# iAmLakshya/code-rag

Hardware: AMD Instinct MI355X
Metric: top-k queries/s over 10Mx768 (cosine top-100, batch 64) (higher is better)
Workload: dtype bf16; 1 GPU; 1x MI355X: 10000000x768 bf16 corpus per GPU resident in HBM, batch-64 queries, exact top-100; rows_per_gpu=10000000, dim=768, batch=64, k=100, parallelism=row-shard x1, hbm_resident_bytes_per_row=2308

## Files before the change

code-rag_amd/csrc/crh_i8.hpp:

```cpp
#pragma once

namespace crh {

typedef __attribute__((ext_vector_type(4))) int i32x4;
typedef __attribute__((ext_vector_type(16))) int i32x16;
typedef __attribute__((ext_vector_type(2))) float f32x2;

constexpr int kI8SampleTiles = 8192;
constexpr float kI8QueryLevels = 16256.0f;

#ifdef CRH_ENABLE_DEBUG
struct I8DebugEnds {
    float *hi, *lo;
    long long pitch;
};
__device__ I8DebugEnds g_i8_debug_ends;
#endif

template <bool F32>
__global__ __launch_bounds__(64) void k_requant_i8(const u32x4 *__restrict__ xt, const float *__restrict__ xf32, u32x4 *__restrict__ x8,
                                                   float *__restrict__ srow, unsigned int *__restrict__ dn_bits, int64_t t0, int ksteps,
                                                   int64_t count, u32x4 *__restrict__ xrow)
{
    const int64_t tile = t0 + blockIdx.x;
    const int lane = threadIdx.x, row = lane & 31, hh = lane >> 5;
    const bool live = tile * 32 + row < count;
    const u32x4 *tp = xt + (size_t)tile * ksteps * 64;
    const int ks8 = ksteps >> 1, dim = ksteps * 16;
    const float4 *fr = reinterpret_cast<const float4 *>(xf32 + ((size_t)tile * 32 + row) * dim);
    auto fetch16 = [&](int p, float (&v)[16], bool copy_row) {
        if (!live) {
#pragma unroll
// ... 117 lines not shown
    }
}

__device__ __forceinline__ uint32_t bf16_bits_up(float x)
{
    const uint32_t u = f32_bits(x);
    return (u >> 31) ? (u >> 16) : ((u + 0xffffu) >> 16);
}
__device__ __forceinline__ int nonsample_tile(int p, int G, int S)
{
    const int per = S - 1, full = G * per;
    if (p >= full) return G * S + (p - full);
    const int blk = p / per;
    return blk * S + 1 + (p - blk * per);
}

template <int KS8, int WAVES, int RING, int QB, int PART>
__global__ __launch_bounds__(WAVES * 64) void k_scan_i8(
    const u32x4 *__restrict__ x8, const float *__restrict__ srow, const unsigned int *__restrict__ dn_bits,
    const u32x4 *__restrict__ qfrag8, const float *__restrict__ qpar, const uint32_t *__restrict__ rowmask, int ntiles, int G, int S,
    uint32_t *__restrict__ gkey, float *__restrict__ tau_g, int k, float c_abs, float sqrt_dim, int nq, u32x4 *__restrict__ wave_lists,
    int wave_cap, unsigned int *__restrict__ qcount, u32x2 *__restrict__ qlist, float *__restrict__ qlo, int qcap,
    SearchStatus *__restrict__ status, const u32x4 *__restrict__ xt, const float *__restrict__ xf32,
    const float *__restrict__ qn, const u32x4 *__restrict__ xrow, u32x4 *__restrict__ shi = nullptr)
{
    static_assert(PART >= 1 && PART <= 3, "sample tiles / thresholds / pass");
    static_assert(KS8 % RING == 0, "the ring must divide the pieces of a tile (slot s % RING holds piece s of every tile)");
    constexpr int NT = WAVES * 64, NQS = QB * 32, NB = NT < 1024 ? NT : 1024;
    __shared__ u32x4 qs[QB * 2 * KS8 * 64];
    __shared__ uint32_t col[kI8SampleTiles];
    __shared__ unsigned int hist[(NT / 64) * 256];
    __shared__ unsigned int bcast[2];
    __shared__ unsigned int fast[NB + 256 + 2 * (NT / 64) + 8];
    __shared__ float tau_s[NQS];
    __shared__ unsigned int qcnt_l[64];
    __shared__ unsigned int wpre[WAVES + 1];
    __shared__ unsigned int wcnt_l[WAVES];
    __shared__ float hwf[64];
    __shared__ int next_m;
    __shared__ unsigned long long cslot[8];
    __shared__ int next_g;
    const int tid = threadIdx.x;
    const int lane = tid & 63;
    const int wave = __builtin_amdgcn_readfirstlane(tid >> 6);
    const int h = lane >> 5;

    CRH_STAMP(0);
    if (tid < 64) qcnt_l[tid] = 0u;
    if (tid < WAVES) wcnt_l[tid] = 0u;
    if (tid == 0) {
        next_m = WAVES;
        next_g = WAVES;
        if constexpr (PART == 3) {
            for (int j = 2; j < 8; ++j) cslot[j] = ~0ull;
            cslot[0] = (unsigned long long)blockIdx.x;
            cslot[1] = (1ull << 32) | (gridDim.x + __hip_atomic_fetch_add(&status->next_chunk, 1u, __ATOMIC_RELAXED, __HIP_MEMORY_SCOPE_AGENT));
        }
// ... 153 lines not shown
                uint32_t m = 0u;
#pragma unroll
                for (int r = 0; r < 16; ++r) {
                    const int row = (r & 3) + 8 * (r >> 2) + 4 * h;
                    const uint32_t key = (ord_f32(lower_end(hi[b][r], sr, b, r)) & ~31u) | (uint32_t)row;
                    m = max(m, ((vmask >> row) & 1u) ? key : 0u);
                }
                m = max(m, (uint32_t)__shfl_xor((int)m, 32));
                if (h == 0) gkey[(size_t)(b * 32 + lane) * G + g] = m;
            }
            g = gn_;
        }
        asm volatile("s_waitcnt vmcnt(0)" ::: "memory");
        return;
    }

    constexpr unsigned int kFloorKey = 0x007fffffu;
    constexpr int SELCAP = 384;
    static_assert(NB + 256 + 2 * (NT / 64) + 8 >= 2 * SELCAP, "sel / selv overlay the scratch of wg_kth_largest_fast");
    static_assert((NT / 64) * 256 >= KS8 * 32, "the canonical query overlays the radix histograms");
    if constexpr (PART == 2)
    for (int q = blockIdx.x; q < NQS; q += gridDim.x) {
        float t = -INFINITY;
        if (q >= nq) {
            t = INFINITY;
        } else if (G >= k) {
            constexpr int DIM = KS8 * 32;
            float qreg[(DIM + NT - 1) / NT];
#pragma unroll
            for (int j = 0; j < (DIM + NT - 1) / NT; ++j) qreg[j] = (tid + j * NT < DIM) ? qn[(size_t)q * DIM + tid + j * NT] : 0.f;
            {
                constexpr int PER = kI8SampleTiles / NT;
                uint32_t kreg[PER];
#pragma unroll
                for (int j = 0; j < PER; ++j) kreg[j] = (tid + j * NT < G) ? gkey[(size_t)q * G + tid + j * NT] : 0u;
#pragma unroll
                for (int j = 0; j < PER; ++j)
                    if (tid + j * NT < G) col[tid + j * NT] = kreg[j];
            }
            __syncthreads();
            CRH_TAU_STAMP(8);
            const uint32_t key = wg_kth_largest_fast<NT, NB, 256>([&](unsigned int i) { return col[i]; }, (unsigned int)G, (unsigned int)k,
                                                                  kFloorKey, fast, hist, bcast);
            __syncthreads();
            CRH_TAU_STAMP(9);
            if (key > kFloorKey) {
// ... 19 lines not shown
                if (nsel <= (unsigned int)SELCAP) {
                    const int sub = tid & 7;
                    for (unsigned int r0 = 0; r0 < nsel; r0 += NT / 8) {
                        const unsigned int r = r0 + (unsigned int)(tid >> 3);
                        float acc = 0.f;
                        if (r < nsel) {
                            const uint32_t e = sel[r];
                            acc = partial_dot8<6>(xt, xf32, xrow, DIM, KS8 * 2, (uint32_t)((e >> 5) * (uint32_t)S * 32u + (e & 31u)), qv, sub);
                        }
                        acc = sum8(acc);
                        if (r < nsel && sub == 0) selv[r] = acc;
                    }
                    __syncthreads();
                    CRH_TAU_STAMP(11);
                    if ((unsigned int)tid < nsel) {
                        const float v = selv[tid];
                        unsigned int gt = 0u, ge = 0u;
                        for (unsigned int j = 0; j < nsel; ++j) {
                            const float o = selv[j];
                            gt += o > v ? 1u : 0u;
                            ge += o >= v ? 1u : 0u;
                        }
                        if (gt < (unsigned int)k && (unsigned int)k <= ge) bcast[1] = f32_bits(v);
                    }
                    __syncthreads();
                    CRH_TAU_STAMP(12);
                    t = fmaxf(t, bits_f32(bcast[1]) - c_abs);
                }
            }
            __syncthreads();
        }
        if (tid == 0) tau_g[q] = t;
    }
    if constexpr (PART == 2) return;
    const bool stored = shi != nullptr;
    const int npass = stored ? ntiles - G : ntiles;
    auto order = [&](int p) { return stored ? nonsample_tile(p, G, S) : p; };
    if (gw < npass) prime(tile_ptr(order(gw)));
    for (int i = tid; i < QB * 2 * KS8 * 64; i += NT) qs[i] = qfrag8[i];
    CRH_STAMP(5);
    if (tid < NQS) tau_s[tid] = tau_g[tid];
    __syncthreads();
    float tq[QB];
#pragma unroll
    for (int b = 0; b < QB; ++b) tq[b] = tau_s[b * 32 + (lane & 31)];

    auto emit_tile = [&](int64_t tile, uint32_t vmask, const float (&hi)[QB][16], uint32_t rounded) __attribute__((always_inline)) {
        uint32_t pmask = 0u;
#pragma unroll
        for (int b = 0; b < QB; ++b)
#pragma unroll
            for (int r = 0; r < 16; ++r) pmask |= (hi[b][r] >= tq[b]) ? (1u << (b * 16 + r)) : 0u;
        {
            const uint32_t t = vmask >> (4 * h);
            const uint32_t v16 = (t & 0xfu) | ((t >> 4) & 0xf0u) | ((t >> 8) & 0xf00u) | ((t >> 12) & 0xf000u);
            pmask &= v16 | (v16 << 16);
        }
#if defined(CRH_I8_DBG) && CRH_I8_DBG == 2
        asm volatile("" ::"v"(pmask));
        pmask = 0u;
#endif
        if (pmask != 0u) {
            const uint32_t rowbase = (uint32_t)(tile * 32) + 4u * (uint32_t)h;
            unsigned int pos = atomicAdd(&wcnt_l[wave], (unsigned int)__popc(pmask));
            uint32_t m = pmask;
            do {
                const int bit = __builtin_ctz(m);
                m &= m - 1u;
                float hv = hi[0][0];
#pragma unroll
                for (int b = 0; b < QB; ++b)
#pragma unroll
                    for (int rr = 0; rr < 16; ++rr) hv = (bit == b * 16 + rr) ? hi[b][rr] : hv;
                const int r = bit & 15;
                if (pos < (unsigned int)wave_cap) {
                    u32x4 e;
                    e.x = f32_bits(hv);
                    e.y = rowbase + (uint32_t)((r & 3) + 8 * (r >> 2));
                    e.z = (uint32_t)((bit >> 4) * 32 + (lane & 31));
                    e.w = rounded;
                    mylist[pos] = e;
                    atomicAdd(&qcnt_l[e.z], 1u);
                }
                ++pos;
            } while (m != 0u);
        }
    };
    if (stored) {
        for (int g = gw; g < G; g += total) {
            float hi[QB][16];
#pragma unroll
            for (int b = 0; b < QB; ++b)
#pragma unroll
                for (int v = 0; v < 2; ++v) {
                    const u32x4 pk = shi[((size_t)g * (QB * 2) + b * 2 + v) * 64 + lane];
                    const uint32_t w4[4] = {pk.x, pk.y, pk.z, pk.w};
#pragma unroll
                    for (int e = 0; e < 4; ++e) {
                        hi[b][8 * v + 2 * e] = bits_f32(w4[e] << 16);
                        hi[b][8 * v + 2 * e + 1] = bits_f32(w4[e] & 0xffff0000u);
                    }
                }
            const int64_t tile = (int64_t)g * S;
            emit_tile(tile, rowmask[tile], hi, 1u);
        }
    }
    int i = gw;
    const u32x4 *xp = tile_ptr(i < npass ? order(i) : 0);
    while (i < npass) {
#if !defined(CRH_I8_STATIC)
        int inext_l = 0;
        if (lane == 0) {
            const int m = atomicAdd(&next_m, 1);
            const unsigned int j = (unsigned int)(m / WAVES), w = (unsigned int)(m % WAVES);
            if (w == 0) {
                const unsigned int c = gridDim.x + __hip_atomic_fetch_add(&status->next_chunk, 1u, __ATOMIC_RELAXED, __HIP_MEMORY_SCOPE_AGENT);
                __hip_atomic_store(&cslot[(j + 1) % 8], ((unsigned long long)(j + 1) << 32) | c, __ATOMIC_RELAXED, __HIP_MEMORY_SCOPE_WORKGROUP);
            }
            unsigned long long e;
            while (((e = __hip_atomic_load(&cslot[j % 8], __ATOMIC_RELAXED, __HIP_MEMORY_SCOPE_WORKGROUP)) >> 32) != j) __builtin_amdgcn_s_sleep(1);
            const unsigned int c = (unsigned int)e;
            inext_l = c > 0x7fffffffu / WAVES ? 0x7fffffff : (int)(c * WAVES + w);
        }
        const int inext = __builtin_amdgcn_readfirstlane(inext_l);
#else
        const int inext = i + total;
#endif
        const int64_t tile = order(i);
        const u32x4 *xn = (inext < npass) ? tile_ptr(order(inext)) : xp;
        const uint32_t vmask = rowmask[tile];
        float sr[32];
#pragma unroll
        for (int j = 0; j < 32; ++j) sr[j] = srow[(size_t)tile * 32 + j];
        i32x16 acc[QB][2];
        scan_tile(xp, xn, acc);
        float hi[QB][16];
        intervals(acc, sr, hi);
        emit_tile(tile, vmask, hi, 0u);
        xp = xn;
        i = inext;
    }
    asm volatile("s_waitcnt vmcnt(0)" ::: "memory");
    CRH_STAMP(6);
#ifdef CRH_FUSED_STAMPS
    if (lane == 0 && blockIdx.x < 256 && wave < 16) g_fused_stamps[256 * 8 + blockIdx.x * 16 + wave] = wall_clock64();
#endif

    if (lane == 0) {
        const unsigned int wcnt = wcnt_l[wave];
        wpre[wave + 1] = wcnt < (unsigned int)wave_cap ? wcnt : (unsigned int)wave_cap;
        atomicMax(&status->max_wave_cnt, wcnt);
        if (wcnt > (unsigned int)wave_cap) atomicAdd(&status->wave_overflow, 1u);
    }
    __syncthreads();
    unsigned int *base = reinterpret_cast<unsigned int *>(qs);
    unsigned int *off = base + 64;
    if (tid < 64) {
        const unsigned int n = qcnt_l[tid];
        base[tid] = n ? atomicAdd(&qcount[tid], n) : 0u;
        off[tid] = 0u;
    }
// ... 24 lines not shown
        }
#pragma unroll
        for (int j = 0; j < 8; ++j) {
            const unsigned int e = e0 + j * NT;
            s_r[j] = e < nall ? srow[cnd[j].y] : 0.f;
        }
#pragma unroll
        for (int j = 0; j < 8; ++j) {
            const unsigned int e = e0 + j * NT;
            if (e < nall) {
                const unsigned int q = cnd[j].z & 63u;
                const unsigned int idx = base[q] + atomicAdd(&off[q], 1u);
                if (idx < (unsigned int)qcap) {
                    u32x2 o;
                    o.x = cnd[j].x;
                    o.y = cnd[j].y;
                    qlist[(size_t)q * qcap + idx] = o;
                    const float up = bits_f32(cnd[j].x);
                    qlo[(size_t)q * qcap + idx] = up - 2.0f * fmaf(s_r[j], hwf[q], c_abs) - 2e-6f - (cnd[j].w ? fabsf(up) * (1.0f / 128.0f) : 0.f);
                }
            }
        }
    }
#ifdef CRH_FUSED_STAMPS
    __syncthreads();
    CRH_STAMP(7);
#endif
}

}
```

code-rag_amd/csrc/crh_index.hip:

```cpp
#include <algorithm>
#include <chrono>
#include <cmath>
#include <cstdlib>
#include <cstring>
#include <vector>

#include "crh_common.h"
#include "crh_kernels.hpp"
#include "crh_i8.hpp"
#include "crh_range.hpp"

namespace crh {
std::string &last_error_ref()
{
    thread_local std::string s;
    return s;
}
}

using namespace crh;

namespace {

constexpr int kWaves = 16;
// ... 46 lines not shown

}

struct crh_index {
    int dim = 0, ksteps = 0, dtype = 0, ncols = 0, device = 0, cu_count = 0;
    int batch_q = 64;
    bool wide_ok = false;
    bool fused_scan = true;
    std::chrono::steady_clock::time_point fused_rest_until{};
    double fused_rest_s = 0.2;
    bool fused_resting() const { return std::chrono::steady_clock::now() < fused_rest_until; }
    bool i8 = false;
    u32x4 *x8 = nullptr;
    float *srow = nullptr;
    u32x4 *xrow = nullptr;
    bool want_xrow = true;
    unsigned int *i8stat = nullptr;
    int64_t x8_cap_tiles = 0, i8_dirty_from = 0;
    int i8_strikes = 0;
    int i8_cooldown = 0;
    bool i8_suppress = false;
    int nominate_max = CRH_NOMINATE_INT8;
    bool i8_sample_record = true;
    bool i8_sample_auto = true;
    int i8_sample = kI8SampleTiles;
    int64_t i8_min_rows = 1000000;
    int64_t cap_rows = 0, cap_tiles = 0, count = 0, alive_count = 0;
    uint64_t mutations = 1;
    MaskCache mask;
    bool sparse_on = true;
    int sparse_den = kSparseDen;
    MaskCache cmask;
    FilterClasses *cmask_classes = nullptr;
    u32x4 *xt = nullptr;
    float *xf32 = nullptr;
    uint32_t *alive = nullptr;
    int32_t *codes = nullptr;
    unsigned int *scratch_u32 = nullptr;

    int seed_tiles = 4096, wave_cap = 2048, qcap = 65536, force_fallback = 0;

    struct Workspace {
        int ws_blocks = 0, ws_wave_cap = 0, ws_qcap = 0, ws_seed = 0;
        int64_t ws_mask_tiles = 0;
        float *qn = nullptr, *gmax = nullptr, *tau = nullptr, *qpar = nullptr, *qlo = nullptr;
        u32x4 *qfrag = nullptr, *qfrag8 = nullptr, *wave_lists = nullptr, *shi = nullptr;
        uint32_t *effmask = nullptr;
        int64_t ws_cmask_tiles = 0;
        uint32_t *cmask = nullptr;
        uint32_t *cunion = nullptr;
        uint32_t *clist = nullptr;
        uint32_t *tilelist = nullptr;
        u32x2 *qlist = nullptr;
        unsigned long long *skeys = nullptr, *skeys2 = nullptr;
    };
    Workspace ws;
    SearchStatus *status = nullptr;
    float *stage_q = nullptr;
    int64_t stage_q_elems = 0;
    float *stage_os = nullptr;
    int64_t *stage_or = nullptr;
    int64_t stage_out_elems = 0;
    unsigned long long *stage_cnt = nullptr;
    int64_t stage_cnt_elems = 0;
    void *stage_in = nullptr;
    int64_t stage_in_bytes = 0;

    std::vector<Pending> pending;
    int next_slot = 0;
// ... 36 lines not shown
    h->stage_in = nullptr;
    h->stage_in_bytes = 0;
    CRH_HIP(hipMalloc(&h->stage_in, (size_t)bytes));
    h->stage_in_bytes = bytes;
    return CRH_OK;
}

int scan_blocks(const crh_index *h, int64_t nitems)
{
    int64_t b = ceil_div(nitems, kWaves);
    if (b > h->cu_count) b = h->cu_count;
    if (b < 1) b = 1;
    return (int)b;
}

int ensure_workspace(crh_index *h, crh_index::Workspace &w, int wave_cap, int qcap)
{
    const int blocks = h->cu_count;
    if (!w.qn) CRH_TRY(dev_alloc(&w.qn, (int64_t)kWideQ * h->dim));
    if (!w.qfrag) CRH_TRY(dev_alloc(&w.qfrag, (int64_t)(kWideQ / 32) * h->ksteps * 64));
    if (!w.tau) CRH_TRY(dev_alloc(&w.tau, kWideQ));
    if (h->i8 && !w.qfrag8) CRH_TRY(dev_alloc(&w.qfrag8, (int64_t)(kMaxQ / 32) * 2 * (h->dim / 32) * 64));
    if (h->i8 && !w.qpar) CRH_TRY(dev_alloc(&w.qpar, kMaxQ * 4));
    if (h->i8 && !w.shi && hipMalloc(reinterpret_cast<void **>(&w.shi), (size_t)kI8SampleTiles * 64 * 4 * sizeof(u32x4)) != hipSuccess) {
        (void)hipGetLastError();
        w.shi = nullptr;
        h->i8_sample_record = false;
    }
    if (!h->status) {
        CRH_TRY(dev_alloc(&h->status, kStatusSlots));
        CRH_HIP(hipMemset(h->status, 0, sizeof(SearchStatus) * kStatusSlots));
    }
    if (w.ws_seed < h->seed_tiles) {
        dev_free(w.gmax);
        w.ws_seed = 0;
        CRH_TRY(dev_alloc(&w.gmax, (int64_t)h->seed_tiles * kWideQ));
        w.ws_seed = h->seed_tiles;
    }
    if (w.ws_mask_tiles < h->cap_tiles) {
        dev_free(w.effmask);
        dev_free(w.tilelist);
        w.ws_mask_tiles = 0;
        h->mask.built_at = 0;
        CRH_TRY(dev_alloc(&w.effmask, h->cap_tiles));
        CRH_TRY(dev_alloc(&w.tilelist, h->cap_tiles + ceil_div(h->cap_tiles, 256) + 1));
        w.ws_mask_tiles = h->cap_tiles;
// ... 365 lines not shown
    }
    return CRH_OK;
}

float i8_c_abs(const crh_index *h) { return 1.5e-4f * (h->dim > 768 ? (float)h->dim / 768.f : 1.f) + 1e-5f; }

void i8_sample_plan(const crh_index *h, int64_t ntiles, int *G, int *S)
{
    int64_t g_auto = h->i8_sample;
    if (h->seed_tiles == 4096 && h->i8_sample_auto)
        g_auto = std::max<int64_t>(1024, std::min<int64_t>(h->i8_sample, (int64_t)(h->i8_sample * std::sqrt((double)ntiles / 312500.0))));
    *G = (int)std::min<int64_t>(h->seed_tiles == 4096 ? g_auto : h->seed_tiles, ntiles);
    *S = (int)std::max<int64_t>(1, ntiles / *G);
}

template <int PART>
int launch_scan_i8(crh_index *h, crh_index::Workspace &w, int blocks, hipStream_t st, const uint32_t *mask, int ntiles, int G, int S, int k, float c_abs,
                   int nq, int wave_cap, int qcap, SearchStatus *stt, u32x4 *shi)
{
#define CRH_I8(KS8, RING, QB)                                                                                                          \
    hipLaunchKernelGGL((k_scan_i8<KS8, kI8Waves, RING, QB, PART>), dim3(PART == 2 ? QB * 32 : blocks), dim3(kI8Waves * 64), 0, st, h->x8, h->srow, \
                       h->i8stat, w.qfrag8, w.qpar, mask, ntiles, G, S, reinterpret_cast<uint32_t *>(w.gmax), w.tau, k, c_abs, sqrtf((float)h->dim), \
                       nq, w.wave_lists, wave_cap, stt->qcount, w.qlist, w.qlo, qcap, stt, h->xt,                                               \
                       h->dtype == CRH_DTYPE_F32 ? h->xf32 : (const float *)nullptr, w.qn, h->xrow, PART == 2 ? (u32x4 *)nullptr : shi)
    switch (h->dim) {
    case 384: CRH_I8(12, 12, 2); break;
    case 768: CRH_I8(24, kI8Ring, 2); break;
    case 1024: CRH_I8(32, kI8Ring, 2); break;
    case 1536: CRH_I8(48, kI8Ring, 1); break;
    default: return fail(CRH_E_INTERNAL, "no int8 scan kernel for dim %d", h->dim);
    }
#undef CRH_I8
    CRH_HIP(hipGetLastError());
    return CRH_OK;
}

template <int MODE>
int launch_scan_wide(crh_index *h, crh_index::Workspace &w, hipStream_t st, const uint32_t *mask, int nitems, int stride, int nblk, int wave_cap, int qcap,
                     SearchStatus *stt)
{
    const int blocks = (int)std::max<int64_t>(1, std::min<int64_t>(nitems, h->cu_count));
#define CRH_WIDE(KS)                                                                                                              \
    hipLaunchKernelGGL((k_scan_wide<KS, MODE>), dim3(blocks), dim3(512), 0, st, h->xt, w.qfrag, w.tau, mask, nitems, stride, nblk, \
                       w.gmax, kWideQ, w.wave_lists, kWideWaves, wave_cap * (kWaves / kWideWaves), stt->qcount, w.qlist, qcap, stt)
    switch (h->ksteps) {
    case 24: CRH_WIDE(24); break;
    case 48: CRH_WIDE(48); break;
// ... 473 lines not shown
    int ndev = 0;
    if (hipGetDeviceCount(&ndev) != hipSuccess || ndev == 0) return fail(CRH_E_NODEVICE, "no HIP device visible");
    if (device < 0 || device >= ndev) return fail(CRH_E_INVALID, "device %d out of range (%d visible)", device, ndev);
    hipDeviceProp_t prop;
    CRH_HIP(hipGetDeviceProperties(&prop, device));
    if (strncmp(prop.gcnArchName, "gfx950", 6) != 0)
        return fail(CRH_E_NODEVICE, "device %d is %s; this library is built for gfx950 only", device, prop.gcnArchName);
    DeviceGuard g(device);
    if (!g.ok) return fail(CRH_E_HIP, "hipSetDevice(%d) failed", device);

    crh_index *h = new crh_index();
    h->dim = dim;
    h->ksteps = dim / 16;
    h->batch_q = dim > 1024 ? 32 : 64;
    h->wide_ok = dim <= 768 && getenv("CODERAG_HIP_NO_WIDE_SCAN") == nullptr;
    {
        const char *e = getenv("CODERAG_HIP_FUSED_SCAN");
        h->fused_scan = !(e && e[0] == '0');
        const char *e8 = getenv("CODERAG_HIP_I8");
        h->i8 = h->fused_scan && !(e8 && e8[0] == '0');
        if (h->i8) h->qcap = 131072;
        if (const char *em = getenv("CODERAG_HIP_I8_MIN_ROWS")) h->i8_min_rows = atoll(em);
        if (const char *er = getenv("CODERAG_HIP_I8_SAMPLE_RECORD")) h->i8_sample_record = !(er[0] == '0');
        if (const char *es = getenv("CODERAG_HIP_I8_SAMPLE")) {
            h->i8_sample = std::max(1024, std::min(kI8SampleTiles, atoi(es)));
            h->i8_sample_auto = false;
        }
        if (const char *er = getenv("CODERAG_HIP_ROWMAJOR")) h->want_xrow = er[0] != '0';
        if (const char *ep = getenv("CODERAG_HIP_SPARSE")) h->sparse_on = ep[0] != '0';
        if (const char *ed = getenv("CODERAG_HIP_SPARSE_DEN")) h->sparse_den = std::max(1, atoi(ed));
    }
    h->dtype = dtype;
    h->ncols = n_code_cols;
    h->device = device;
    h->cu_count = prop.multiProcessorCount;
    h->cap_rows = (capacity_rows + 31) & ~31LL;
    h->cap_tiles = h->cap_rows / 32;
    int rc = dev_alloc(&h->xt, h->cap_tiles * h->ksteps * 64);
    if (rc == CRH_OK && dtype == CRH_DTYPE_F32) rc = dev_alloc(&h->xf32, h->cap_rows * dim);
    if (rc == CRH_OK) rc = dev_alloc(&h->alive, h->cap_tiles);
    if (rc == CRH_OK && n_code_cols) rc = dev_alloc(&h->codes, h->cap_rows * n_code_cols);
    if (rc == CRH_OK) rc = dev_alloc(&h->scratch_u32, 4);
    if (rc == CRH_OK && hipMemset(h->xt, 0, (size_t)h->cap_tiles * h->ksteps * 1024) != hipSuccess) rc = fail(CRH_E_HIP, "hipMemset(xt) failed");
    if (rc == CRH_OK && hipMemset(h->alive, 0, (size_t)h->cap_tiles * 4) != hipSuccess) rc = fail(CRH_E_HIP, "hipMemset(alive) failed");
    if (rc == CRH_OK && h->codes && hipMemset(h->codes, 0xff, (size_t)h->cap_rows * n_code_cols * 4) != hipSuccess)
        rc = fail(CRH_E_HIP, "hipMemset(codes) failed");
// ... 15 lines not shown
    dev_free(h->xf32);
    dev_free(h->alive);
    dev_free(h->codes);
    dev_free(h->scratch_u32);
    dev_free(h->mask.sets);
    dev_free(h->cmask.sets);
    dev_free(h->cmask_classes);
    {
        crh_index::Workspace &w = h->ws;
        dev_free(w.qn);
        dev_free(w.gmax);
        dev_free(w.tau);
        dev_free(w.qfrag);
        dev_free(w.wave_lists);
        dev_free(w.effmask);
        dev_free(w.tilelist);
        dev_free(w.cmask);
        dev_free(w.cunion);
        dev_free(w.clist);
        dev_free(w.qlist);
        dev_free(w.skeys);
        dev_free(w.qfrag8);
        dev_free(w.shi);
        dev_free(w.qpar);
        dev_free(w.qlo);
        dev_free(w.skeys2);
    }
    dev_free(h->x8);
    dev_free(h->srow);
    dev_free(h->xrow);
    dev_free(h->i8stat);
    dev_free(h->status);
    dev_free(h->stage_q);
    dev_free(h->stage_os);
    dev_free(h->stage_or);
    dev_free(h->stage_cnt);
    if (h->stage_in) (void)hipFree(h->stage_in);
    for (auto &e : h->ev) (void)hipEventDestroy(e);
    delete h;
    return CRH_OK;
}

static int append_impl(crh_index *h, int64_t n, const float *vecs, int on_device, const int32_t *codes, int64_t *first_row_out,
                       void *stream, int preprocessed);

int crh_index_append(crh_index *h, int64_t n, const float *vecs, int on_device, const int32_t *codes, int64_t *first_row_out,
// ... 493 lines not shown
                    for (int lane = 0; lane < 64; ++lane)
                        for (int e = 0; e < 8; ++e) {
                            const uint32_t word = rec[((((size_t)t * QB + blk) * 2 + v) * 64 + lane) * 4 + (e >> 1)];
                            const uint32_t bits = (e & 1) ? (word & 0xffff0000u) : (word << 16);
                            const int r = 8 * v + e, q = blk * 32 + (lane & 31);
                            const int64_t row = t * 32 + (r & 3) + 8 * (r >> 2) + 4 * (lane >> 5);
                            if (q < b && row < count) memcpy(hi_rec_out + (int64_t)(q0 + q) * count + row, &bits, 4);
                        }
        int G8, S8;
        i8_sample_plan(h, ntiles, &G8, &S8);
        u32x4 *shi = h->i8_sample_record ? w.shi : nullptr;
        CRH_TRY(launch_scan_i8<1>(h, w, blocks, st, mask.mask, (int)ntiles, G8, S8, k, c_abs, b, wave_cap, qcap, stt, shi));
        CRH_TRY(launch_scan_i8<2>(h, w, blocks, st, mask.mask, (int)ntiles, G8, S8, k, c_abs, b, wave_cap, qcap, stt, shi));
        CRH_HIP(hipDeviceSynchronize());
        CRH_HIP(hipMemcpy(tau_out + q0, w.tau, (size_t)b * 4, hipMemcpyDeviceToHost));
        CRH_HIP(hipMemcpy(qpar_out + (int64_t)q0 * 4, w.qpar, (size_t)b * 16, hipMemcpyDeviceToHost));
    }
    for (int64_t i = (int64_t)nq * 4; i < (int64_t)kMaxQ * 4; ++i) qpar_out[i] = 0.f;
    CRH_HIP(hipMemcpy(srow_out, h->srow, (size_t)count * 4, hipMemcpyDeviceToHost));
    CRH_HIP(hipMemcpy(dn_out, h->i8stat, 4, hipMemcpyDeviceToHost));
    *c_abs_out = c_abs;
    return CRH_OK;
}
#endif

#ifdef CRH_FUSED_STAMPS
int crh_debug_fused_stamps(unsigned long long *out)
{
    CRH_HIP(hipDeviceSynchronize());
    CRH_HIP(hipMemcpyFromSymbol(out, HIP_SYMBOL(g_fused_stamps), sizeof(unsigned long long) * 256 * 24));
    return CRH_OK;
}
int crh_debug_select_stamps(unsigned long long *out)
{
    CRH_HIP(hipDeviceSynchronize());
    CRH_HIP(hipMemcpyFromSymbol(out, HIP_SYMBOL(g_select_stamps), sizeof(unsigned long long) * 64 * 16));
    return CRH_OK;
}
#endif

int crh_index_set_nomination(crh_index *h, int mode)
{
    if (!h) return fail(CRH_E_INVALID, "index is NULL");
    if (mode < CRH_NOMINATE_BF16_3 || mode > CRH_NOMINATE_INT8) return fail(CRH_E_INVALID, "unknown nomination mode %d", mode);
    h->nominate_max = mode;
    if (mode == CRH_NOMINATE_INT8) h->i8_strikes = h->i8_cooldown = 0;
// ... 249 lines not shown
```

code-rag_amd/ffi.py:

```python

from __future__ import annotations

import ctypes as C
import os
from pathlib import Path

import numpy as np

PKG_DIR = Path(__file__).resolve().parent
LIB_PATH = Path(os.environ.get("CODERAG_HIP_LIB", PKG_DIR / "lib" / "libcoderag_hip.so"))

OK, E_INVALID, E_HIP, E_CAPACITY, E_NODEVICE, E_INTERNAL = 0, -1, -2, -3, -4, -5
DTYPE_F32, DTYPE_BF16 = 0, 1
NOMINATE_BF16_3, NOMINATE_BF16, NOMINATE_INT8 = 0, 1, 2
MAX_FILTERS, MAX_K = 8, 1024
MAX_LISTS = 16
FUSE_RRF, FUSE_MAX = 0, 1
FUSE_METHODS = {"rrf": FUSE_RRF, "max": FUSE_MAX}
MAX_POS, MAX_NEG = 8, 8
RECOMMEND_AVERAGE, RECOMMEND_BEST = 0, 1
RECOMMEND_STRATEGIES = {"average": RECOMMEND_AVERAGE, "best": RECOMMEND_BEST}
COND_IN, COND_NOT_IN, COND_BETWEEN, COND_NOT_BETWEEN = 0, 1, 2, 3
RANGE_MODES = {"between": COND_BETWEEN, "not_between": COND_NOT_BETWEEN}
VALUE_MAX = 2 ** 31 - 1
# ... 3 lines not shown

EXPORTS = (
    "crh_abi_version", "crh_last_error", "crh_device_count", "crh_device_info",
    "crh_index_create", "crh_index_destroy", "crh_index_append", "crh_index_append_preprocessed", "crh_index_tombstone",
    "crh_index_tombstone_filter", "crh_index_compact", "crh_index_export", "crh_index_import",
    "crh_index_count", "crh_index_clear", "crh_index_reserve", "crh_index_read_rows",
    "crh_search", "crh_search_finish", "crh_search_get_stats", "crh_index_set_tuning",
    "crh_index_set_nomination", "crh_index_get_nomination",
    "crh_merge_topk", "crh_merge_topk_strided", "crh_index_match_rows", "crh_index_set_profiling", "crh_index_get_profile",
    "crh_search_cond", "crh_index_match_rows_cond", "crh_index_tombstone_cond", "crh_index_set_sparse_route",
    "crh_gemm_bf16_bias", "crh_gemm_bf16_bias_res_ln", "crh_gemm_bf16_res_lnstats", "crh_gemm_bf16_lnin", "crh_layernorm_apply", "crh_gemm_bf16_bias_res32_ln", "crh_attn_fwd_varlen", "crh_embed_ln",
    "crh_masked_mean_pool", "crh_gather_rows_i32", "crh_gather_rows_bytes", "crh_gather_rerank_columns", "crh_rerank_vector",
    "crh_embed_ln_packed", "crh_attn_fwd_packed", "crh_masked_mean_pool_packed", "crh_encoder_finish",
    "crh_index_gather_vectors", "crh_mmr_select",
    "crh_index_gather_codes", "crh_group_select",
    "crh_search_multi",
    "crh_fuse_select",
    "crh_recommend_query", "crh_recommend_select",
    "crh_search_range",
    "crh_span_select",
    "crh_index_row_mask", "crh_lex_create", "crh_lex_destroy", "crh_lex_clear", "crh_lex_count", "crh_lex_append", "crh_lex_stats",
    "crh_lex_search",
)
DEBUG_EXPORTS = ("crh_debug_gemm_variant", "crh_debug_read_ceiling", "crh_debug_i8_move", "crh_debug_i8_intervals")
DEBUG_LIB_PATH = Path(os.environ.get("CODERAG_HIP_DEBUG_LIB", PKG_DIR / "lib" / "libcoderag_hip_debug.so"))

RR_NAME_BYTES, RR_MAX_ENTITIES, RR_ENTITY_BYTES = 64, 8, 48


class NativeError(RuntimeError):
    def __init__(self, code: int, message: str):
        super().__init__(f"libcoderag_hip error {code}: {message}")
        self.code = code


class Filter(C.Structure):
    _fields_ = [("col", C.c_int32), ("code", C.c_int32)]


class Condition(C.Structure):
    _fields_ = [("col", C.c_int32), ("negate", C.c_int32), ("n", C.c_int64), ("codes", C.c_void_p)]


class RerankQuery(C.Structure):
    _fields_ = [("vector_weight", C.c_double), ("centrality_weight", C.c_double), ("n_entities", C.c_int32),
                ("entity_len", C.c_int32 * 8), ("entity", (C.c_uint8 * 48) * 8), ("pad_", C.c_int32)]

# ... 104 lines not shown
    L.crh_rerank_vector.argtypes = [i32, i32, vp, vp, C.POINTER(RerankColumns), vp, C.c_double, i32, i32, i32, vp, vp, vp, vp, vp, vp]
    L.crh_index_gather_vectors.argtypes = [vp, i64, vp, i64, vp, vp]
    L.crh_mmr_select.argtypes = [i32, i32, i32, i32, vp, vp, vp, C.c_float, vp, vp, vp, vp, vp]
    L.crh_index_gather_codes.argtypes = [vp, i32, i64, vp, i64, vp, vp]
    L.crh_group_select.argtypes = [i32, i32, i32, i32, vp, vp, vp, vp, vp, vp, vp, vp, vp]
    L.crh_span_select.argtypes = [i32, i32, i32, i32, vp, vp, vp, vp, vp, vp, vp, vp, vp, vp, vp, vp, vp]
    L.crh_fuse_select.argtypes = [i32, i32, i32, i32, i32, i32, vp, vp, vp, vp, vp, vp, vp, vp, vp, vp]
    L.crh_recommend_query.argtypes = [i32, i32, i32, i32, vp, vp, vp, vp, vp]
    L.crh_recommend_select.argtypes = [i32, i32, i32, i32, i32, i32, i32, i32, vp, vp, vp, vp, vp, vp, vp, vp, vp, vp, vp, vp, vp]
    L.crh_index_row_mask.argtypes = [vp, C.POINTER(Condition), i32, vp, i64, vp]
    L.crh_lex_create.argtypes = [i32, i64, C.POINTER(vp)]
    L.crh_lex_destroy.argtypes = [vp]
    L.crh_lex_clear.argtypes = [vp]
    L.crh_lex_count.argtypes = [vp, C.POINTER(i64), C.POINTER(i64)]
    L.crh_lex_append.argtypes = [vp, i64, vp, vp, vp, vp]
    L.crh_lex_stats.argtypes = [vp, vp, i64, vp, vp, C.POINTER(i64), C.POINTER(i64)]
    L.crh_lex_search.argtypes = [vp, i32, vp, vp, vp, C.c_float, C.c_float, C.c_float, i32, vp, i64, vp, vp, vp, vp]
    if debug or hasattr(L, "crh_debug_gemm_variant"):
        debug = True
        L.crh_debug_gemm_variant.argtypes = [vp, vp, vp, vp, i32, i32, i32, i32, vp]
        L.crh_debug_read_ceiling.argtypes = [vp, vp]
        L.crh_debug_i8_move.argtypes = [vp]
        L.crh_debug_i8_intervals.argtypes = [vp, i32, vp, i32, C.POINTER(Filter), i32, vp, vp, vp, vp, vp, vp, vp, vp]
    for name in EXPORTS + (DEBUG_EXPORTS if debug else ()):
        if name != "crh_last_error":
            getattr(L, name).restype = i32
    if L.crh_abi_version() != ABI_VERSION:
        raise NativeError(E_INTERNAL, f"ABI version mismatch between ffi.py and {path.name}")
    return L


def check(rc: int, L: C.CDLL | None = None) -> None:
    if rc != OK:
        raise NativeError(rc, ((L or lib()).crh_last_error() or b"").decode("utf-8", "replace"))


def use_device(device: int) -> None:
    import torch
    if torch.cuda.is_available() and torch.cuda.current_device() != int(device):
        torch.cuda.set_device(int(device))


def current_stream(device) -> int:
    import torch
    return int(torch.cuda.current_stream(device).cuda_stream)

# ... 88 lines not shown
    if len(classes) <= MAX_CLASSES:
        return classes, qclass, [np.arange(qclass.size)]
    order = np.argsort(qclass, kind="stable")
    group = qclass[order] // MAX_CLASSES
    return classes, qclass, [order[group == g] for g in range((len(classes) + MAX_CLASSES - 1) // MAX_CLASSES)]


def multi_passes(class_filters, query_class, batch_q: int = 64) -> int:
    return sum((len(c) + batch_q - 1) // batch_q for c in multi_plan(class_filters, query_class)[2])


def debug_i8_intervals(handle, rows: int, dim: int, queries, k: int, filters=None) -> dict:
    q = np.ascontiguousarray(queries, dtype=np.float32).reshape(-1, dim)
    nq = q.shape[0]
    out = {"hi_rec": np.empty((nq, rows), np.float32), "hi": np.empty((nq, rows), np.float32), "lo": np.empty((nq, rows), np.float32),
           "srow": np.empty((rows,), np.float32), "qpar": np.empty((64, 4), np.float32), "dn": np.empty((1,), np.float32),
           "c_abs": np.empty((1,), np.float32), "tau": np.empty((nq,), np.float32)}
    farr, nf = _filters(filters)
    L = debug_lib()
    check(L.crh_debug_i8_intervals(handle, nq, q.ctypes.data, int(k), farr, nf, *(out[n].ctypes.data for n in
                                   ("hi_rec", "hi", "lo", "srow", "qpar", "dn", "c_abs", "tau"))), L)
    out["dn"], out["c_abs"] = np.float32(out["dn"][0]), np.float32(out["c_abs"][0])
    return out


def range_thresholds(thresholds, nq: int) -> np.ndarray:
    thr = np.asarray(thresholds, dtype=np.float32)
    thr = np.full((nq,), thr, np.float32) if thr.ndim == 0 else np.ascontiguousarray(thr.reshape(-1))
    if thr.shape[0] != nq:
        raise NativeError(E_INVALID, f"{thr.shape[0]} thresholds for {nq} queries")
    if not np.isfinite(thr).all():
        raise NativeError(E_INVALID, "a score threshold must be a finite number")
    return thr


def _has_sets(filters) -> bool:
    return any(is_set_condition(item) for item in (filters or []))


def _ptr(x) -> int:
    if x is None:
        return None
    if isinstance(x, int):
        return x
    if isinstance(x, np.ndarray):
        return x.ctypes.data
# ... 746 lines not shown
```

include/coderag_hip.h:

```cpp
#ifndef CODERAG_HIP_H
#define CODERAG_HIP_H

#include <stdint.h>

#ifdef __cplusplus
extern "C" {
#endif

#define CRH_ABI_VERSION 4

#define CRH_OK 0
#define CRH_E_INVALID (-1)
#define CRH_E_HIP (-2)
#define CRH_E_CAPACITY (-3)
#define CRH_E_NODEVICE (-4)
#define CRH_E_INTERNAL (-5)

#define CRH_DTYPE_F32 0
#define CRH_DTYPE_BF16 1

#define CRH_MAX_FILTERS 8
#define CRH_MAX_K 1024

typedef struct crh_index crh_index;
// ... 238 lines not shown
                 uint64_t *kmask, int B, int L, int D, void *stream);

int crh_masked_mean_pool(const void *tok, const uint64_t *kmask, float *sent, int B, int L, int D,
                         void *stream);

int crh_embed_ln_packed(const int32_t *ids, const int32_t *row_off, const void *word, const void *pos, const void *type0,
                        const float *gamma, const float *beta, float eps, int pad_id, void *out, uint64_t *kmask, int B,
                        int T, int Lmax, int D, void *stream);
int crh_attn_fwd_packed(const void *qkv, const int32_t *row_off, const uint64_t *kmask, void *out, int B, int T, int Lmax,
                        int H, void *stream);
int crh_masked_mean_pool_packed(const void *tok, const int32_t *row_off, const uint64_t *kmask, float *sent, int B, int T,
                                int Lmax, int D, void *stream);
int crh_encoder_finish(void *stream);

#ifdef CRH_ENABLE_DEBUG
int crh_debug_read_ceiling(crh_index *h, void *stream);

int crh_debug_i8_move(crh_index *h);

int crh_debug_i8_intervals(crh_index *h, int nq, const float *queries, int k, const crh_filter *filters, int n_filters,
                           float *hi_rec_out, float *hi_out, float *lo_out, float *srow_out, float *qpar_out, float *dn_out,
                           float *c_abs_out, float *tau_out);

int crh_debug_gemm_variant(const void *x, const void *w, const float *bias, void *y, int T, int N, int K,
                           int variant, void *stream);

#endif

#ifdef __cplusplus
}
#endif
#endif
```

Before: 48330 queries/s per 10M-row shard (row.query pairs/s / 1e7).

## Raise int8 scan pruning thresholds dynamically from candidate lower-bound counts

During the int8 scan pass, each emitted candidate's guaranteed lower bound is binned against per-query levels taken from the sample phase (the k/2, k/4, ... order statistics). Waves periodically flush these counts to global atomics. Once at least k candidates are known to exceed a level, the shared per-query threshold is raised with atomicMax, so later tiles nominate fewer candidates for exact rescoring. This adds shared and global atomics, per-tile smax reductions and flush overhead in the hot loop, and it relies on the lower-bound bound being correct.

```diff
diff --git a/code-rag_amd/csrc/crh_i8.hpp b/code-rag_amd/csrc/crh_i8.hpp
--- a/code-rag_amd/csrc/crh_i8.hpp
+++ b/code-rag_amd/csrc/crh_i8.hpp
@@ -8,6 +8,8 @@
 
 constexpr int kI8SampleTiles = 8192;
 constexpr float kI8QueryLevels = 16256.0f;
+constexpr int kI8RiseLevels = 8;
+constexpr int kI8RiseLevel = 0, kI8RiseCount = 64 * kI8RiseLevels, kI8RiseTau = 2 * 64 * kI8RiseLevels, kI8RiseWords = kI8RiseTau + 64;
 
 #ifdef CRH_ENABLE_DEBUG
 struct I8DebugEnds {
@@ -171,7 +173,8 @@
     uint32_t *__restrict__ gkey, float *__restrict__ tau_g, int k, float c_abs, float sqrt_dim, int nq, u32x4 *__restrict__ wave_lists,
     int wave_cap, unsigned int *__restrict__ qcount, u32x2 *__restrict__ qlist, float *__restrict__ qlo, int qcap,
     SearchStatus *__restrict__ status, const u32x4 *__restrict__ xt, const float *__restrict__ xf32,
-    const float *__restrict__ qn, const u32x4 *__restrict__ xrow, u32x4 *__restrict__ shi = nullptr)
+    const float *__restrict__ qn, const u32x4 *__restrict__ xrow, u32x4 *__restrict__ shi = nullptr, unsigned int *__restrict__ rise = nullptr,
+    int rising = 0)
 {
     static_assert(PART >= 1 && PART <= 3, "sample tiles / thresholds / pass");
     static_assert(KS8 % RING == 0, "the ring must divide the pieces of a tile (slot s % RING holds piece s of every tile)");
@@ -181,7 +184,9 @@
     __shared__ unsigned int hist[(NT / 64) * 256];
     __shared__ unsigned int bcast[2];
     __shared__ unsigned int fast[NB + 256 + 2 * (NT / 64) + 8];
-    __shared__ float tau_s[NQS];
+    __shared__ unsigned int tau_o[NQS];
+    __shared__ float lev_s[64 * kI8RiseLevels];
+    __shared__ unsigned int cnt_l[kI8RiseLevels * 64];
     __shared__ unsigned int qcnt_l[64];
     __shared__ unsigned int wpre[WAVES + 1];
     __shared__ unsigned int wcnt_l[WAVES];
@@ -381,6 +386,7 @@
     if constexpr (PART == 2)
     for (int q = blockIdx.x; q < NQS; q += gridDim.x) {
         float t = -INFINITY;
+        if (tid < kI8RiseLevels) lev_s[tid] = INFINITY;
         if (q >= nq) {
             t = INFINITY;
         } else if (G >= k) {
@@ -446,6 +452,13 @@
                             ge += o >= v ? 1u : 0u;
                         }
                         if (gt < (unsigned int)k && (unsigned int)k <= ge) bcast[1] = f32_bits(v);
+                        if (rising) {
+#pragma unroll
+                            for (int j = 0; j < kI8RiseLevels; ++j) {
+                                const unsigned int rj = (unsigned int)max(1, k >> (j + 1));
+                                if (gt < rj && rj <= ge) lev_s[j] = v - c_abs;
+                            }
+                        }
                     }
                     __syncthreads();
                     CRH_TAU_STAMP(12);
@@ -455,6 +468,13 @@
             __syncthreads();
         }
         if (tid == 0) tau_g[q] = t;
+        if (rise != nullptr) {
+            if (tid < kI8RiseLevels) {
+                reinterpret_cast<float *>(rise + kI8RiseLevel)[q * kI8RiseLevels + tid] = lev_s[tid];
+                rise[kI8RiseCount + tid * 64 + q] = 0u;
+            }
+            if (tid == 0) reinterpret_cast<float *>(rise + kI8RiseTau)[q] = t;
+        }
     }
     if constexpr (PART == 2) return;
     const bool stored = shi != nullptr;
@@ -463,18 +483,21 @@
     if (gw < npass) prime(tile_ptr(order(gw)));
     for (int i = tid; i < QB * 2 * KS8 * 64; i += NT) qs[i] = qfrag8[i];
     CRH_STAMP(5);
-    if (tid < NQS) tau_s[tid] = tau_g[tid];
+    if (tid < NQS) tau_o[tid] = ord_f32(tau_g[tid]);
+    for (int i = tid; i < kI8RiseLevels * 64; i += NT) {
+        cnt_l[i] = 0u;
+        lev_s[i] = (rising && i < NQS * kI8RiseLevels) ? reinterpret_cast<const float *>(rise + kI8RiseLevel)[i] : INFINITY;
+    }
     __syncthreads();
-    float tq[QB];
-#pragma unroll
-    for (int b = 0; b < QB; ++b) tq[b] = tau_s[b * 32 + (lane & 31)];
-
-    auto emit_tile = [&](int64_t tile, uint32_t vmask, const float (&hi)[QB][16], uint32_t rounded) __attribute__((always_inline)) {
+
+    auto emit_tile = [&](int64_t tile, uint32_t vmask, const float (&hi)[QB][16], uint32_t rounded, uint32_t smax_bits) __attribute__((always_inline)) {
         uint32_t pmask = 0u;
 #pragma unroll
-        for (int b = 0; b < QB; ++b)
-#pragma unroll
-            for (int r = 0; r < 16; ++r) pmask |= (hi[b][r] >= tq[b]) ? (1u << (b * 16 + r)) : 0u;
+        for (int b = 0; b < QB; ++b) {
+            const float tq = unord_f32(tau_o[b * 32 + (lane & 31)]);
+#pragma unroll
+            for (int r = 0; r < 16; ++r) pmask |= (hi[b][r] >= tq) ? (1u << (b * 16 + r)) : 0u;
+        }
         {
             const uint32_t t = vmask >> (4 * h);
             const uint32_t v16 = (t & 0xfu) | ((t >> 4) & 0xf0u) | ((t >> 8) & 0xf00u) | ((t >> 12) & 0xf000u);
@@ -505,9 +528,35 @@
                     e.w = rounded;
                     mylist[pos] = e;
                     atomicAdd(&qcnt_l[e.z], 1u);
+                    if (rising && rounded == 0u) {
+                        const float lo_c = hv - 2.0f * fmaf(bits_f32(smax_bits), hwf[e.z], c_abs) - 2e-6f;
+                        int lv = -1;
+#pragma unroll
+                        for (int j = 0; j < kI8RiseLevels; ++j) lv = (lo_c >= lev_s[e.z * kI8RiseLevels + j]) ? j : lv;
+                        if (lv >= 0) atomicAdd(&cnt_l[lv * 64 + (int)e.z], 1u);
+                    }
                 }
                 ++pos;
             } while (m != 0u);
+        }
+    };
+    auto flush_levels = [&]() __attribute__((always_inline)) {
+        if (lane < NQS) {
+            unsigned int reach = 0u;
+            int top = -1;
+#pragma unroll
+            for (int j = kI8RiseLevels - 1; j >= 0; --j) {
+                const unsigned int c = atomicExch(&cnt_l[j * 64 + lane], 0u);
+                unsigned int *dc = rise + kI8RiseCount + j * 64 + lane;
+                reach += c ? __hip_atomic_fetch_add(dc, c, __ATOMIC_RELAXED, __HIP_MEMORY_SCOPE_AGENT) + c
+                           : __hip_atomic_load(dc, __ATOMIC_RELAXED, __HIP_MEMORY_SCOPE_AGENT);
+                top = (top < 0 && reach >= (unsigned int)k) ? j : top;
+            }
+            if (top >= 0) {
+                const float lv = lev_s[lane * kI8RiseLevels + top];
+                if (lv < INFINITY) atomicMax(&tau_o[lane], ord_f32(lv));
+            }
+            reinterpret_cast<float *>(rise + kI8RiseTau)[lane] = unord_f32(__hip_atomic_load(&tau_o[lane], __ATOMIC_RELAXED, __HIP_MEMORY_SCOPE_WORKGROUP));
         }
     };
     if (stored) {
@@ -526,17 +575,18 @@
                     }
                 }
             const int64_t tile = (int64_t)g * S;
-            emit_tile(tile, rowmask[tile], hi, 1u);
+            emit_tile(tile, rowmask[tile], hi, 1u, 0u);
         }
     }
     int i = gw;
     const u32x4 *xp = tile_ptr(i < npass ? order(i) : 0);
     while (i < npass) {
 #if !defined(CRH_I8_STATIC)
-        int inext_l = 0;
+        int inext_l = 0, flush_l = 0;
         if (lane == 0) {
             const int m = atomicAdd(&next_m, 1);
             const unsigned int j = (unsigned int)(m / WAVES), w = (unsigned int)(m % WAVES);
+            flush_l = (w == 0 && ((j & (j - 1u)) == 0u || (j & 15u) == 0u)) ? 1 : 0;
             if (w == 0) {
                 const unsigned int c = gridDim.x + __hip_atomic_fetch_add(&status->next_chunk, 1u, __ATOMIC_RELAXED, __HIP_MEMORY_SCOPE_AGENT);
                 __hip_atomic_store(&cslot[(j + 1) % 8], ((unsigned long long)(j + 1) << 32) | c, __ATOMIC_RELAXED, __HIP_MEMORY_SCOPE_WORKGROUP);
@@ -547,6 +597,7 @@
             inext_l = c > 0x7fffffffu / WAVES ? 0x7fffffff : (int)(c * WAVES + w);
         }
         const int inext = __builtin_amdgcn_readfirstlane(inext_l);
+        if (rising && __builtin_amdgcn_readfirstlane(flush_l)) flush_levels();
 #else
         const int inext = i + total;
 #endif
@@ -560,7 +611,10 @@
         scan_tile(xp, xn, acc);
         float hi[QB][16];
         intervals(acc, sr, hi);
-        emit_tile(tile, vmask, hi, 0u);
+        uint32_t smax_bits = 0u;
+#pragma unroll
+        for (int j = 0; j < 32; ++j) smax_bits = max(smax_bits, f32_bits(sr[j]));
+        emit_tile(tile, vmask, hi, 0u, smax_bits);
         xp = xn;
         i = inext;
     }
@@ -631,6 +685,7 @@
             }
         }
     }
+    if (rising && wave == 0) flush_levels();
 #ifdef CRH_FUSED_STAMPS
     __syncthreads();
     CRH_STAMP(7);
diff --git a/code-rag_amd/csrc/crh_index.hip b/code-rag_amd/csrc/crh_index.hip
--- a/code-rag_amd/csrc/crh_index.hip
+++ b/code-rag_amd/csrc/crh_index.hip
@@ -92,6 +92,7 @@
     bool i8_suppress = false;
     int nominate_max = CRH_NOMINATE_INT8;
     bool i8_sample_record = true;
+    bool i8_rising = true;
     bool i8_sample_auto = true;
     int i8_sample = kI8SampleTiles;
     int64_t i8_min_rows = 1000000;
@@ -115,6 +116,7 @@
         int64_t ws_mask_tiles = 0;
         float *qn = nullptr, *gmax = nullptr, *tau = nullptr, *qpar = nullptr, *qlo = nullptr;
         u32x4 *qfrag = nullptr, *qfrag8 = nullptr, *wave_lists = nullptr, *shi = nullptr;
+        unsigned int *rise = nullptr;
         uint32_t *effmask = nullptr;
         int64_t ws_cmask_tiles = 0;
         uint32_t *cmask = nullptr;
@@ -197,6 +199,10 @@
     if (!w.tau) CRH_TRY(dev_alloc(&w.tau, kWideQ));
     if (h->i8 && !w.qfrag8) CRH_TRY(dev_alloc(&w.qfrag8, (int64_t)(kMaxQ / 32) * 2 * (h->dim / 32) * 64));
     if (h->i8 && !w.qpar) CRH_TRY(dev_alloc(&w.qpar, kMaxQ * 4));
+    if (h->i8 && !w.rise) {
+        CRH_TRY(dev_alloc(&w.rise, kI8RiseWords));
+        CRH_HIP(hipMemset(w.rise, 0, sizeof(unsigned int) * kI8RiseWords));
+    }
     if (h->i8 && !w.shi && hipMalloc(reinterpret_cast<void **>(&w.shi), (size_t)kI8SampleTiles * 64 * 4 * sizeof(u32x4)) != hipSuccess) {
         (void)hipGetLastError();
         w.shi = nullptr;
@@ -608,7 +614,8 @@
     hipLaunchKernelGGL((k_scan_i8<KS8, kI8Waves, RING, QB, PART>), dim3(PART == 2 ? QB * 32 : blocks), dim3(kI8Waves * 64), 0, st, h->x8, h->srow, \
                        h->i8stat, w.qfrag8, w.qpar, mask, ntiles, G, S, reinterpret_cast<uint32_t *>(w.gmax), w.tau, k, c_abs, sqrtf((float)h->dim), \
                        nq, w.wave_lists, wave_cap, stt->qcount, w.qlist, w.qlo, qcap, stt, h->xt,                                               \
-                       h->dtype == CRH_DTYPE_F32 ? h->xf32 : (const float *)nullptr, w.qn, h->xrow, PART == 2 ? (u32x4 *)nullptr : shi)
+                       h->dtype == CRH_DTYPE_F32 ? h->xf32 : (const float *)nullptr, w.qn, h->xrow, PART == 2 ? (u32x4 *)nullptr : shi, w.rise,     \
+                       h->i8_rising ? 1 : 0)
     switch (h->dim) {
     case 384: CRH_I8(12, 12, 2); break;
     case 768: CRH_I8(24, kI8Ring, 2); break;
@@ -1128,6 +1135,7 @@
         if (h->i8) h->qcap = 131072;
         if (const char *em = getenv("CODERAG_HIP_I8_MIN_ROWS")) h->i8_min_rows = atoll(em);
         if (const char *er = getenv("CODERAG_HIP_I8_SAMPLE_RECORD")) h->i8_sample_record = !(er[0] == '0');
+        if (const char *er = getenv("CODERAG_HIP_I8_RISING")) h->i8_rising = !(er[0] == '0');
         if (const char *es = getenv("CODERAG_HIP_I8_SAMPLE")) {
             h->i8_sample = std::max(1024, std::min(kI8SampleTiles, atoi(es)));
             h->i8_sample_auto = false;
@@ -1189,6 +1197,7 @@
         dev_free(w.skeys);
         dev_free(w.qfrag8);
         dev_free(w.shi);
+        dev_free(w.rise);
         dev_free(w.qpar);
         dev_free(w.qlo);
         dev_free(w.skeys2);
@@ -1728,6 +1737,24 @@
     *c_abs_out = c_abs;
     return CRH_OK;
 }
+
+int crh_debug_i8_rising(crh_index *h, int on, float *tau_out, unsigned int *counts_out)
+{
+    if (!h) return fail(CRH_E_INVALID, "index is NULL");
+    DeviceGuard g(h->device);
+    if (!g.ok) return fail(CRH_E_HIP, "hipSetDevice(%d) failed", h->device);
+    CRH_HIP(hipDeviceSynchronize());
+    if (on == 0 || on == 1) h->i8_rising = on == 1;
+    if (!tau_out && !counts_out) return CRH_OK;
+    if (!h->ws.rise) return fail(CRH_E_INVALID, "no int8-nominated batch has run on this index");
+    unsigned int rec[kI8RiseWords];
+    CRH_HIP(hipMemcpy(rec, h->ws.rise, sizeof(rec), hipMemcpyDeviceToHost));
+    if (tau_out) memcpy(tau_out, rec + kI8RiseTau, 64 * sizeof(float));
+    if (counts_out)
+        for (int q = 0; q < 64; ++q)
+            for (int j = 0; j < kI8RiseLevels; ++j) counts_out[q * kI8RiseLevels + j] = rec[kI8RiseCount + j * 64 + q];
+    return CRH_OK;
+}
 #endif
 
 #ifdef CRH_FUSED_STAMPS
diff --git a/code-rag_amd/ffi.py b/code-rag_amd/ffi.py
--- a/code-rag_amd/ffi.py
+++ b/code-rag_amd/ffi.py
@@ -49,7 +49,7 @@
     "crh_index_row_mask", "crh_lex_create", "crh_lex_destroy", "crh_lex_clear", "crh_lex_count", "crh_lex_append", "crh_lex_stats",
     "crh_lex_search",
 )
-DEBUG_EXPORTS = ("crh_debug_gemm_variant", "crh_debug_read_ceiling", "crh_debug_i8_move", "crh_debug_i8_intervals")
+DEBUG_EXPORTS = ("crh_debug_gemm_variant", "crh_debug_read_ceiling", "crh_debug_i8_move", "crh_debug_i8_intervals", "crh_debug_i8_rising")
 DEBUG_LIB_PATH = Path(os.environ.get("CODERAG_HIP_DEBUG_LIB", PKG_DIR / "lib" / "libcoderag_hip_debug.so"))
 
 RR_NAME_BYTES, RR_MAX_ENTITIES, RR_ENTITY_BYTES = 64, 8, 48
@@ -200,6 +200,7 @@
         L.crh_debug_read_ceiling.argtypes = [vp, vp]
         L.crh_debug_i8_move.argtypes = [vp]
         L.crh_debug_i8_intervals.argtypes = [vp, i32, vp, i32, C.POINTER(Filter), i32, vp, vp, vp, vp, vp, vp, vp, vp]
+        L.crh_debug_i8_rising.argtypes = [vp, i32, vp, vp]
     for name in EXPORTS + (DEBUG_EXPORTS if debug else ()):
         if name != "crh_last_error":
             getattr(L, name).restype = i32
@@ -334,6 +335,16 @@
                                    ("hi_rec", "hi", "lo", "srow", "qpar", "dn", "c_abs", "tau"))), L)
     out["dn"], out["c_abs"] = np.float32(out["dn"][0]), np.float32(out["c_abs"][0])
     return out
+
+
+def debug_i8_rising(handle, on: int = -1, read: bool = True):
+    L = debug_lib()
+    if not read:
+        check(L.crh_debug_i8_rising(handle, int(on), None, None), L)
+        return None
+    tau, counts = np.empty((64,), np.float32), np.empty((64, 8), np.uint32)
+    check(L.crh_debug_i8_rising(handle, int(on), tau.ctypes.data, counts.ctypes.data), L)
+    return tau, counts
 
 
 def range_thresholds(thresholds, nq: int) -> np.ndarray:
diff --git a/include/coderag_hip.h b/include/coderag_hip.h
--- a/include/coderag_hip.h
+++ b/include/coderag_hip.h
@@ -284,6 +284,8 @@
                            float *hi_rec_out, float *hi_out, float *lo_out, float *srow_out, float *qpar_out, float *dn_out,
                            float *c_abs_out, float *tau_out);
 
+int crh_debug_i8_rising(crh_index *h, int on, float *tau_out, unsigned int *counts_out);
+
 int crh_debug_gemm_variant(const void *x, const void *w, const float *bias, void *y, int T, int N, int K,
                            int variant, void *stream);
 
```

New measurement: 47290 queries/s per 10M-row shard (row.query pairs/s / 1e7). -2.1%, worse.
